# feixue94/pram

Hardware: AMD Instinct MI355X
Metric: query images/sec (640x480, 2048 kpts, 7Scenes nc113) (higher is better)
Workload: dtype f32 results via split-fp16 MFMA (f16 x3 products, f32 accumulate); 1 GPU; 7Scenes full hot path: SFD2 extract+sample -> SegNetViT nc113 (15 layers) -> GML match + 20 Sinkhorn iters, 2048 query kpts vs a 2048-kpt reference set; stages=erm; precision=x3, batches_in_flight_per_gpu=3, hipgraph_replay=False, attention_chunk_keys=4096, frame=640x480, keypoints=2048, parallelism=query-sharded x1, one all-gather of result records, matches_last_step=14291, matches_correct_last_step=14288, gather_order_verified=True

## Files before the change

include/pram_hip.h:

```cpp
#ifndef PRAM_HIP_H
#define PRAM_HIP_H

#include <stddef.h>
#include <stdint.h>

#ifdef __cplusplus
extern "C" {
#endif

#define PRAM_OK 0
#define PRAM_E_ARG (-1)
#define PRAM_E_LAUNCH (-2)
#define PRAM_E_UNSUPPORTED (-3)

int pram_hip_version(void);
const char* pram_last_error(void);
const char* pram_last_kernel(void);

#define PRAM_STATUS_X3_RANGE 1u
int pram_set_status_word(unsigned int* device_word);
float pram_x3_set_act_scale(float scale);
int pram_read_status_word(unsigned int* host_out, int reset, void* stream);


// ... 194 lines not shown

int pram_sample_nhwc_f32(const float* fmap, int batch, int fh, int fw, int c, const float* kpts,
                         const int* lens, int n_max, int s, int l2norm, float* out, void* stream);


int pram_sfd2_row_list(const float* kpts, const int* lens, int batch, int n_max, int fh, int fw, int s, int* rows,
                       int* n_rows, int* pix2row, int rlen, void* stream);

int pram_conv3x3_rows_x3_f32(const float* in, int batch, int h, int w, int cin, const void* wgt_hi, const void* wgt_lo,
                             float w_scale, const float* bias, const int* rows, const int* n_rows, int rlen, float* out,
                             int cout, int relu, void* stream);

int pram_conv1x1_rows_x3_l2norm_f32(const float* in, int batch, int rlen, int cin, const void* wgt_hi, const void* wgt_lo,
                                    float w_scale, const float* bias, const int* n_rows, float* out, int cout, void* stream);

int pram_sample_rows_f32(const float* rowmap, const int* pix2row, int batch, int rlen, int fh, int fw, int c, const float* kpts,
                         const int* lens, int n_max, int s, int l2norm, float* out, void* stream);

int pram_l2norm_rows_f32(float* x, int rows, int cols, void* stream);

int pram_score_lookup_f32(const float* score_map, long long map_stride, int h, int w, const float* kpts,
                          const int* lens, int batch, int n_max, float* out, void* stream);


int pram_resize_bilinear_f32(const float* in, float* out, int planes, int h, int w, int oh, int ow,
                             void* stream);

int pram_seg_epilogue_f32(const float* logits, const int* lens, int batch, int n_max, int n_class,
                          float bg_threshold, float* seg_scores, int* seg_ids, int* non_bg_mask,
                          int* n_non_bg, void* stream);
// ... 251 lines not shown
```

pram_amd/_lib.py:

```python
from __future__ import annotations

import ctypes as C
from pathlib import Path

import os as _os
_LIB_PATH = Path(_os.environ["PRAM_HIP_LIB"]) if _os.environ.get("PRAM_HIP_LIB") else Path(__file__).resolve().parent / "csrc" / "libpram_hip.so"
_lib = None

P = C.c_void_p
I = C.c_int
F = C.c_float
LL = C.c_longlong
SZ = C.c_size_t

_SIGS = {
    "pram_hip_version": (I, []),
    "pram_last_error": (C.c_char_p, []),
    "pram_last_kernel": (C.c_char_p, []),
    "pram_set_status_word": (I, [P]),
    "pram_read_status_word": (I, [P, I, P]),
    "pram_x3_set_act_scale": (F, [F]),
    "pram_linear_f32": (I, [P, I, I, P, I, I, P, P, P, I, P, I, I, I, F, I, P, P, I, P]),
    "pram_linear_f16_f32": (I, [P, I, I, P, I, I, P, P, P, I, P, I, I, I, F, I, P, P, I, P]),
    "pram_linear_f16_ragged_f32": (I, [P, I, I, P, I, I, P, P, P, I, P, I, I, I, F, I, P, P, I, P, I, P]),
# ... 46 lines not shown
    "pram_conv2d_nhwc_f32": (I, [P, I, I, I, I, P, P, P, P, P, P, I, I, I, I, P]),
    "pram_conv2d_nhwc_f16_f32": (I, [P, I, I, I, I, P, P, P, P, P, P, I, I, I, I, P]),
    "pram_conv3x3_grouped_nhwc_f32": (I, [P, I, I, I, I, P, P, P, P, I, I, P]),
    "pram_image_to_nhwc4_f32": (I, [P, P, I, I, I, P]),
    "pram_nhwc_to_nchw_f32": (I, [P, P, I, I, I, I, P]),
    "pram_score_map_f32": (I, [P, P, I, I, I, P]),
    "pram_simple_nms_workspace_bytes": (SZ, [I, I, I]),
    "pram_simple_nms_f32": (I, [P, P, I, I, I, I, P, P]),
    "pram_select_keypoints_workspace_bytes": (SZ, [I, I, I, I]),
    "pram_select_keypoints_f32": (I, [P, I, I, I, F, I, I, I, I, P, P, P, P, P]),
    "pram_sample_nhwc_f32": (I, [P, I, I, I, I, P, P, I, I, I, P, P]),
    "pram_l2norm_rows_f32": (I, [P, I, I, P]),
    "pram_sfd2_row_list": (I, [P, P, I, I, I, I, I, P, P, P, I, P]),
    "pram_conv3x3_rows_x3_f32": (I, [P, I, I, I, I, P, P, F, P, P, P, I, P, I, I, P]),
    "pram_conv1x1_rows_x3_l2norm_f32": (I, [P, I, I, I, P, P, F, P, P, P, I, P]),
    "pram_sample_rows_f32": (I, [P, P, I, I, I, I, I, P, P, I, I, I, P, P]),
    "pram_resize_bilinear_f32": (I, [P, P, I, I, I, I, I, P]),
    "pram_seg_epilogue_f32": (I, [P, P, I, I, I, F, P, P, P, P, P]),
    "pram_row_sort_desc_f32": (I, [P, I, I, I, P, P, P]),
    "pram_row_top2_f32": (I, [P, I, LL, P, P, I, I, I, I, P, P, P, P]),
    "pram_proj_dist_top2_f32": (I, [P, I, P, P, I, I, F, P, P, P, P]),
    "pram_proj_dist_top2_f64uv": (I, [P, I, P, P, I, I, I, C.c_double, P, P, P, P]),
    "pram_project_points_f64": (I, [P, P, P, I, C.c_double, C.c_double, P, P, P, P, P, P]),
    "pram_seg_vote": (I, [P, P, I, I, I, P, P, P, P, P, P, P]),
    "pram_pack_record_f32": (I, [P, P, P, P, P, I, I, I, P, P]),
    "pram_fill_u32": (I, [P, C.c_uint, SZ, P]),
    "pram_stage_frames_u8": (I, [P, P, P, I, I, I, P]),
    "pram_score_lookup_f32": (I, [P, LL, I, I, P, P, I, I, P, P]),
    "pram_cand_mask_ranks": (I, [P, P, I, I, I, P]),
    "pram_cand_plan": (I, [P, P, P, P, P, I, I, I, I, P, P, P, I, I, P, P, P, P, I, I, C.c_double, I, P, P]),
# ... 80 lines not shown
```

pram_amd/csrc/conv.hip:

```cpp
#include <stdlib.h>
#include "gemm_core.h"
#include "gemm_core_f16.h"
#include "gemm_core_x3.h"
#include "gemm_core_x3w.h"
#include "launch.h"

namespace {

struct ConvArgs {
    const float* in; const float* w; const float* bias; const float* scale; const float* shift;
    const float* residual; float* out;
    int batch, h, wd, cin, cout, ks, stride, relu;
    int ho, wo, m, k;
    int tiles_m, tiles_n;
    unsigned int* status;
    _Float16* out_hi; _Float16* out_lo;
    float act_scale = gemmx3::ACT_SCALE;
    const int* rows = nullptr; const int* n_rows = nullptr; int rlen = 0;
};

constexpr int ROWS_BM = 256;

template <int MI, int WN>
__device__ __forceinline__ void conv_epilogue(const ConvArgs& p, f32x16 (&acc)[MI][2], int row0, int col0, int BM, int BN) {
// ... 31 lines not shown
            }
            if (full) {
#pragma unroll
                for (int e = 0; e < 16; ++e) p.out[(size_t)(rbase + acc_row(mi, e, h)) * p.cout + col] = q[e];
            } else {
#pragma unroll
                for (int e = 0; e < 16; ++e) {
                    const int row = rbase + acc_row(mi, e, h);
                    if (row < p.m && col < p.cout) p.out[(size_t)row * p.cout + col] = q[e];
                }
            }
        }
    }
}

template <int MI, int WN>
__device__ __forceinline__ void conv_epilogue_l2norm(const ConvArgs& p, f32x16 (&acc)[MI][2], int row0, int col0, int BM, float* scratch) {
    using gemm::acc_row;
    const int tid = threadIdx.x;
    const int lane = tid & 63, wave = tid >> 6;
    const int wm = wave / WN, wn = wave % WN;
    const int r = lane & 31, h = lane >> 5;
    const int nlast = p.cout - 1, mlast = p.m - 1;
    const int rloc = wm * 32 * MI;
    const int rbase = row0 + rloc;
#pragma unroll
    for (int ni = 0; ni < 2; ++ni) {
        const int col = col0 + wn * 64 + ni * 32 + r;
        const int cc = min(col, nlast);
        const float bi = p.bias ? p.bias[cc] : 0.f;
        const float sc = p.scale ? p.scale[cc] : 1.f;
        const float sh = p.scale ? p.shift[cc] : 0.f;
#pragma unroll
        for (int mi = 0; mi < MI; ++mi)
#pragma unroll
            for (int e = 0; e < 16; ++e) {
                float v = acc[mi][ni][e] + bi;
                if (p.scale) v = v * sc + sh;
                if (p.residual) v += p.residual[(size_t)min(rbase + acc_row(mi, e, h), mlast) * p.cout + cc];
                if (p.relu) v = fmaxf(v, 0.f);
                acc[mi][ni][e] = col < p.cout ? v : 0.f;
            }
    }
    __syncthreads();
#pragma unroll
    for (int mi = 0; mi < MI; ++mi)
#pragma unroll
        for (int e = 0; e < 16; ++e) {
            float s = acc[mi][0][e] * acc[mi][0][e] + acc[mi][1][e] * acc[mi][1][e];
            s += __builtin_bit_cast(float, __builtin_amdgcn_update_dpp(0, __builtin_bit_cast(int, s), 0xB1, 0xF, 0xF, false));
            s += __builtin_bit_cast(float, __builtin_amdgcn_update_dpp(0, __builtin_bit_cast(int, s), 0x4E, 0xF, 0xF, false));
            s += __builtin_bit_cast(float, __builtin_amdgcn_update_dpp(0, __builtin_bit_cast(int, s), 0x141, 0xF, 0xF, false));
            s += __builtin_bit_cast(float, __builtin_amdgcn_update_dpp(0, __builtin_bit_cast(int, s), 0x140, 0xF, 0xF, false));
            s += __shfl_xor(s, 16, 64);
            if (r == 0) scratch[wn * BM + rloc + acc_row(mi, e, h)] = s;
        }
    __syncthreads();
#pragma unroll
    for (int mi = 0; mi < MI; ++mi)
#pragma unroll
        for (int e = 0; e < 16; ++e) {
            const int tr = rloc + acc_row(mi, e, h);
            float tot = 0.f;
#pragma unroll
            for (int w = 0; w < WN; ++w) tot += scratch[w * BM + tr];
            const float d = fmaxf(sqrtf(tot), 1e-12f);
            const int row = row0 + tr;
#pragma unroll
            for (int ni = 0; ni < 2; ++ni) {
                const int col = col0 + wn * 64 + ni * 32 + r;
                if (row < p.m && col < p.cout) p.out[(size_t)row * p.cout + col] = acc[mi][ni][e] / d;
            }
        }
}

template <int MI, int WN>
__device__ __forceinline__ void conv_epilogue_planes(const ConvArgs& p, f32x16 (&acc)[MI][2], int row0, int col0, int BM, int BN) {
    const int tid = threadIdx.x;
    const int lane = tid & 63, wave = tid >> 6;
    const int wm = wave / WN, wn = wave % WN;
    const int r = lane & 31, h = lane >> 5;
    const int nlast = p.cout - 1, mlast = p.m - 1;
    const int rbase = row0 + wm * 32 * MI;
    const bool full = (row0 + BM <= p.m) && (col0 + BN <= p.cout);
    const bool odd = lane & 1;
    unsigned int* plane = reinterpret_cast<unsigned int*>(odd ? p.out_lo : p.out_hi);
    const unsigned int sel = odd ? 0x03020706u : 0x05040100u;
    const unsigned int hc = (unsigned int)p.cout >> 1;
// ... 220 lines not shown
    auto okb = [&](int pp, int kt) -> bool { return (col0 + brow + 64 * pp) < p.cout; };
    f32x16 acc[MI][2];
    float amax = 0.f;
    mainloop<MI, WN>(smem, adv, la, oka, lb, okb, p.k / BK, p.act_scale, acc, amax);
    x3_range_flag(p.status, amax);
#pragma unroll
    for (int mi = 0; mi < MI; ++mi)
#pragma unroll
        for (int ni = 0; ni < 2; ++ni)
#pragma unroll
            for (int e = 0; e < 16; ++e) acc[mi][ni][e] *= inv;
    if constexpr (L2N) conv_epilogue_l2norm<MI, WN>(p, acc, row0, col0, BM, reinterpret_cast<float*>(&smem));
    else conv_epilogue<MI, WN>(p, acc, row0, col0, BM, BN);
}

template <int MI, int WM, int WN, bool PLANES = false, bool GATHER = false>
__global__ __launch_bounds__(64 * WM * WN, 2) void conv_x3w_kernel(ConvArgs p, const _Float16* __restrict__ wh,
                                                                    const _Float16* __restrict__ wl, float inv) {
    using namespace gemmx3w;
    using C = Cfg<MI, WM, WN>;
    constexpr int BM = C::BM, BN = C::BN;
    extern __shared__ __attribute__((aligned(16))) unsigned char smem_raw[];
    Smem<MI, WM, WN>& smem = *reinterpret_cast<Smem<MI, WM, WN>*>(smem_raw);
    const int nblk = p.tiles_m * p.tiles_n;
    const int id = xcd_remap(blockIdx.x, nblk);
    const int tn = id % p.tiles_n, tm = id / p.tiles_n;
    const int tid = threadIdx.x;
    const int arow = tid >> 3, akq = tid & 7, qrow = tid >> 2, qsl = tid & 3;
    const int row0 = tm * BM, col0 = tn * BN;
    const int pad = p.ks >> 1;
    int seg = 0, seg_row0 = 0, live = 0;
// ... 44 lines not shown
        const unsigned off = in ? (unsigned)(roff[pp] + tap) : 0u;
        return *reinterpret_cast<const float4*>(base[pp] + off);
    };
    auto oka = [&](int pp, int kt) -> bool {
        const int iy = iy0[pp] + cky, ix = ix0[pp] + ckx;
        return ok[pp] && (unsigned)iy < (unsigned)p.h && (unsigned)ix < (unsigned)p.wd;
    };
    auto lb = [&](int pp, int kt, int plane) -> uint4 { return *reinterpret_cast<const uint4*>((plane ? wl : wh) + boff[pp] + koff); };
    auto okb = [&](int pp, int kt) -> bool { return (col0 + qrow + C::RQ * pp) < p.cout; };
    f32x16 acc[MI][2];
    auto aptr = [](int, int, int) -> const _Float16* { return nullptr; };
    auto bptr = [&](int row, int plane, int kt) -> const _Float16* {
        return (plane ? wl : wh) + (size_t)min(col0 + row, nlast) * p.k + koff;
    };
    float amax = 0.f;
    mainloop<MI, WM, WN, false, 0, 1>(smem, adv, la, oka, lb, okb, aptr, bptr, p.k / BK, p.act_scale, acc, amax);
    x3_range_flag(p.status, amax);
#pragma unroll
    for (int mi = 0; mi < MI; ++mi)
#pragma unroll
        for (int ni = 0; ni < 2; ++ni)
#pragma unroll
            for (int e = 0; e < 16; ++e) acc[mi][ni][e] *= inv;
    if constexpr (PLANES) conv_epilogue_planes<MI, WN>(p, acc, row0, col0, BM, BN);
    else conv_epilogue<MI, WN>(p, acc, row0, col0, BM, BN);
}

namespace halo {
constexpr int TH = 8, TW = 32, HWD = TW + 2, HHT = TH + 2, HP = HWD * HHT;
constexpr int BK = 32, NT = 512;
constexpr int NL = (HP * 8 + NT - 1) / NT;
template <int WN_>
struct alignas(16) Smem {
    _Float16 ah[2][HP * BK];
    _Float16 al[2][HP * BK];
    _Float16 bh[2][WN_ * 64 * BK];
    _Float16 bl[2][WN_ * 64 * BK];
};
}

template <int WN>
__global__ __launch_bounds__(halo::NT, 1) void conv3x3_x3h_kernel(ConvArgs p, const _Float16* __restrict__ wh, const _Float16* __restrict__ wl,
                                                                  float inv, int tiles_x, int tiles_y) {
    using namespace halo;
    using gemmx3::half4;
    using gemmx3::half8;
    constexpr int BN = WN * 64, MI = TH / (NT / 64 / WN);
    extern __shared__ __attribute__((aligned(16))) unsigned char smem_raw[];
    Smem<WN>& s = *reinterpret_cast<Smem<WN>*>(smem_raw);
    const int nblk = p.tiles_m * p.tiles_n;
    const int id = xcd_remap(blockIdx.x, nblk);
    const int tn = id % p.tiles_n;
    int t = id / p.tiles_n;
    const int tx = t % tiles_x; t /= tiles_x;
    const int ty = t % tiles_y;
    const int b = t / tiles_y;
// ... 31 lines not shown
            float4 v = hv[j];
            if (!g.inimg) v = make_float4(0.f, 0.f, 0.f, 0.f);
            half4 hi, lo;
            gemmx3::split4(v, p.act_scale, hi, lo, amax);
            if (g.valid) {
                const int off = g.hp * BK + gemmx3::swz(g.q >> 1, g.hp) * 8 + (g.q & 1) * 4;
                *reinterpret_cast<half4*>(&s.ah[buf][off]) = hi;
                *reinterpret_cast<half4*>(&s.al[buf][off]) = lo;
            }
        }
    };
    auto bdma = [&](int buf, int koff) {
        auto bp = [&](int row, int plane) { return (plane ? wl : wh) + (size_t)min(col0 + row, nlast) * p.k + koff; };
        gemmx3w::dma_tile<BN, NT / 64>(s.bh[buf], s.bl[buf], bp);
    };
    f32x16 acc[MI][2];
#pragma unroll
    for (int mi = 0; mi < MI; ++mi)
#pragma unroll
        for (int ni = 0; ni < 2; ++ni)
#pragma unroll
            for (int e = 0; e < 16; ++e) acc[mi][ni][e] = 0.f;
    auto kstep = [&](int abuf, int bbuf, int ky, int kx, int ks) {
        const int brow0 = (wn * 64 + r) * BK;
        const int bslot = gemmx3::swz(2 * ks + h, r) * 8;
        half8 bh[2], bl[2], ah[2], al[2];
#pragma unroll
        for (int ni = 0; ni < 2; ++ni) {
            bh[ni] = *reinterpret_cast<const half8*>(&s.bh[bbuf][brow0 + ni * 32 * BK + bslot]);
            bl[ni] = *reinterpret_cast<const half8*>(&s.bl[bbuf][brow0 + ni * 32 * BK + bslot]);
        }
        auto aoff = [&](int mi) {
            const int hp = (wm * MI + mi + ky) * HWD + r + kx;
            return hp * BK + gemmx3::swz(2 * ks + h, hp) * 8;
        };
        int o = aoff(0);
        ah[0] = *reinterpret_cast<const half8*>(&s.ah[abuf][o]);
        al[0] = *reinterpret_cast<const half8*>(&s.al[abuf][o]);
// ... 8 lines not shown
#pragma unroll
            for (int ni = 0; ni < 2; ++ni) acc[mi][ni] = __builtin_amdgcn_mfma_f32_32x32x16_f16(al[mi & 1], bh[ni], acc[mi][ni], 0, 0, 0);
#pragma unroll
            for (int ni = 0; ni < 2; ++ni) acc[mi][ni] = __builtin_amdgcn_mfma_f32_32x32x16_f16(ah[mi & 1], bl[ni], acc[mi][ni], 0, 0, 0);
#pragma unroll
            for (int ni = 0; ni < 2; ++ni) acc[mi][ni] = __builtin_amdgcn_mfma_f32_32x32x16_f16(ah[mi & 1], bh[ni], acc[mi][ni], 0, 0, 0);
        }
    };
    const int nslab = p.cin / BK;
    hload(0);
    bdma(0, 0);
    hcommit(0);
    asm volatile("s_waitcnt vmcnt(0)" ::: "memory");
    __syncthreads();
    int c = 0;
    for (int slab = 0; slab < nslab; ++slab) {
        const bool more_slab = slab + 1 < nslab;
#pragma unroll 1
        for (int tap = 0; tap < 9; ++tap, ++c) {
            const int ky = tap / 3, kx = tap - ky * 3;
            const bool more = tap < 8 || more_slab;
            if (more) {
                const int nt = tap < 8 ? tap + 1 : 0, ns = tap < 8 ? slab : slab + 1;
                bdma((c + 1) & 1, nt * p.cin + ns * BK);
            }
            const bool fetch = tap == 0 && more_slab;
            if (fetch) hload(slab + 1);
            __builtin_amdgcn_sched_barrier(0);
            kstep(slab & 1, c & 1, ky, kx, 0);
            kstep(slab & 1, c & 1, ky, kx, 1);
            __builtin_amdgcn_sched_barrier(0);
            if (tap == 8 && more_slab) hcommit((slab + 1) & 1);
            if (fetch) asm volatile("s_waitcnt vmcnt(%0)" ::"n"(NL) : "memory");
            else asm volatile("s_waitcnt vmcnt(0)" ::: "memory");
            __syncthreads();
        }
    }
    x3_range_flag(p.status, amax);
    const int rbase = wm * 32 * MI;
    float* out_b = p.out + (size_t)b * p.ho * p.wo * p.cout;
    const float* res_b = p.residual ? p.residual + (size_t)b * p.ho * p.wo * p.cout : nullptr;
#pragma unroll
    for (int ni = 0; ni < 2; ++ni) {
        const int col = col0 + wn * 64 + ni * 32 + r;
        const int cc = min(col, nlast);
        const float bi = p.bias ? p.bias[cc] : 0.f;
        const float sc = p.scale ? p.scale[cc] : 1.f;
        const float sh = p.scale ? p.shift[cc] : 0.f;
#pragma unroll
        for (int mi = 0; mi < MI; ++mi)
#pragma unroll
            for (int e = 0; e < 16; ++e) {
                const int tr = rbase + gemm::acc_row(mi, e, h);
                const int oy = oy0 + (tr >> 5), ox = ox0 + (tr & 31);
                if (oy < p.ho && ox < p.wo && col < p.cout) {
// ... 325 lines not shown
    PRAM_REQUIRE(batch >= 0 && rlen > 0 && rlen % ROWS_BM == 0 && (long long)batch * rlen < (1ll << 31),
                 "%s: rlen=%d must be a positive multiple of %d (batch * rlen < 2^31)", who, rlen, ROWS_BM);
    p.batch = 1; p.h = 1; p.wd = batch * rlen; p.cin = cin; p.cout = cout; p.ks = 1; p.stride = 1; p.relu = 0;
    if (int e = conv_args(who, p, CONV_X3, in && wgt_hi && wgt_lo && out && n_rows, w_scale)) return e;
    PRAM_REQUIRE(cout > 0 && cout <= 128, "%s: cout=%d must be at most 128", who, cout);
    if (batch == 0) return PRAM_OK;
    const float inv = arm_split(p, w_scale);
    p.n_rows = n_rows; p.rlen = rlen;
    p.tiles_m = cdiv(p.m, gemmx3::Cfg<2, 2>::BM);
    p.tiles_n = 1;
    hipLaunchKernelGGL((conv_x3_kernel<2, 2, true, true>), dim3(p.tiles_m), dim3(gemmx3::NT), 0, (hipStream_t)stream, p,
                       (const _Float16*)wgt_hi, (const _Float16*)wgt_lo, inv);
    return pram_launch_status(who);
}

extern "C" int pram_conv2d_nhwc_x3_planes(const float* in, int batch, int h, int w, int cin, const void* wgt_hi, const void* wgt_lo,
                                          float w_scale, const float* bias, const float* scale, const float* shift,
                                          const float* residual, void* out_hi, void* out_lo, int cout, int ks, int stride, int relu,
                                          void* stream) {
    const char* who = "pram_conv2d_nhwc_x3_planes";
    ConvArgs p{};
    p.in = in; p.bias = bias; p.scale = scale; p.shift = shift; p.residual = residual;
    p.batch = batch; p.h = h; p.wd = w; p.cin = cin; p.cout = cout; p.ks = ks; p.stride = stride; p.relu = relu;
    if (int e = conv_args(who, p, CONV_X3, in && wgt_hi && wgt_lo && out_hi && out_lo, w_scale)) return e;
    PRAM_REQUIRE(cout > 0 && cout % 2 == 0, "%s: cout=%d must be even", who, cout);
    if (batch == 0) return PRAM_OK;
    const float inv = arm_split(p, w_scale);
    p.out_hi = (_Float16*)out_hi;
    p.out_lo = (_Float16*)out_lo;
    using CW = gemmx3w::Cfg<4, 2, 4>;
// ... 226 lines not shown
```

pram_amd/nets/sfd2.py:

```python
from __future__ import annotations

from typing import Dict, List, Optional

import torch
import torch.nn as nn

from .. import ops
from . import _blocks as blk

RGB_mean = [0.485, 0.456, 0.406]
RGB_std = [0.229, 0.224, 0.225]


def norm_RGB(img: torch.Tensor) -> torch.Tensor:
    mean = img.new_tensor(RGB_mean).view(-1, 1, 1)
    std = img.new_tensor(RGB_std).view(-1, 1, 1)
    return (img - mean) / std


def _conv_bn(cin, cout, stride=1):
    return nn.Sequential(nn.Conv2d(cin, cout, 3, stride, 1), nn.BatchNorm2d(cout), nn.ReLU(inplace=True))


class _Res(nn.Module):
# ... 50 lines not shown
            P[name + ".s"], P[name + ".t"] = self._bn(sd, name + ".1")
        for i in range(3):
            p = f"conv4.{i}"
            for j in (1, 2, 3):
                P[f"{p}.w{j}"] = self._ohwi(sd[f"{p}.conv{j}.weight"])
                P[f"{p}.s{j}"], P[f"{p}.t{j}"] = self._bn(sd, f"{p}.bn{j}")
        for head in ("convPa", "convDa"):
            P[head + ".w0"] = self._ohwi(sd[head + ".0.weight"])
            P[head + ".b0"] = sd[head + ".0.bias"].float()
            P[head + ".s0"], P[head + ".t0"] = self._bn(sd, head + ".1")
            P[head + ".w3"] = self._ohwi(sd[head + ".3.weight"])
            P[head + ".b3"] = sd[head + ".3.bias"].float()
        for head in ("convPb", "convDb"):
            P[head + ".w"] = self._ohwi(sd[head + ".weight"])
            P[head + ".b"] = sd[head + ".bias"].float()
        return {k: v.contiguous().to(dev) for k, v in P.items()}

    def _backbone(self, image: torch.Tensor):
        blk.require_cuda(image, "ResNet4x")
        P = self._packed_get(self._build_packed)
        fused1 = ops.gemm_prec() in ("x3", "f16")
        x = image.float().contiguous() if fused1 and image.shape[-1] != 4 else ops.image_to_nhwc4(image.float())

        def cbr(x, n, stride=1):
            return ops.conv2d_nhwc(x, P[n + ".w"], P[n + ".b"], P[n + ".s"], P[n + ".t"], ks=3, stride=stride, relu=True)

        if fused1:
            o1b = ops.sfd2_conv1(x, P["conv1a.w"], P["conv1a.b"], P["conv1a.s"], P["conv1a.t"],
                                 P["conv1b.w"], P["conv1b.b"], P["conv1b.s"], P["conv1b.t"])
        else:
# ... 6 lines not shown
            if ops.GROUPED_X3 and ops.gemm_prec() == "x3" and o4.shape[-1] % 64 == 0 and o4.numel() < (1 << 29):
                yh, yl = ops.conv2d_nhwc_planes(o4, P[p + ".w1"], None, P[p + ".s1"], P[p + ".t1"], ks=1, relu=True)
                y = ops.conv3x3_grouped_planes(yh, yl, P[p + ".w2"], P[p + ".s2"], P[p + ".t2"], groups=o4.shape[-1] // 8, relu=True)
            else:
                y = ops.conv2d_nhwc(o4, P[p + ".w1"], None, P[p + ".s1"], P[p + ".t1"], ks=1, relu=True)
                y = ops.conv3x3_grouped_nhwc(y, P[p + ".w2"], P[p + ".s2"], P[p + ".t2"], groups=32, relu=True)
            o4 = ops.conv2d_nhwc(y, P[p + ".w3"], None, P[p + ".s3"], P[p + ".t3"], residual=o4, ks=1, relu=True)
        return P, o1b, o2b, o3b, o4

    def _score_head(self, P, o4):
        pa = ops.conv2d_nhwc(o4, P["convPa.w0"], P["convPa.b0"], P["convPa.s0"], P["convPa.t0"], ks=3, stride=2, relu=True)
        pa = ops.conv2d_nhwc(pa, P["convPa.w3"], P["convPa.b3"], ks=3)
        logits = ops.conv2d_nhwc(pa, P["convPb.w"], P["convPb.b"], ks=1)
        return logits, ops.score_map(logits)

    def _desc_stem(self, P, o4):
        return ops.conv2d_nhwc(o4, P["convDa.w0"], P["convDa.b0"], P["convDa.s0"], P["convDa.t0"], ks=3, relu=True)

    def _desc_head(self, P, o4):
        da = ops.conv2d_nhwc(self._desc_stem(P, o4), P["convDa.w3"], P["convDa.b3"], ks=3)
        return ops.conv2d_nhwc(da, P["convDb.w"], P["convDb.b"], ks=1, l2norm=True)

    @staticmethod
    def _nchw_view(x_nhwc: torch.Tensor) -> torch.Tensor:
        return x_nhwc.permute(0, 3, 1, 2)

    @torch.no_grad()
    @blk.with_model_precision
    def det(self, x):
        P, _, _, _, o4 = self._backbone(x)
        _, score = self._score_head(P, o4)
        return score, self._nchw_view(self._desc_head(P, o4))

    @torch.no_grad()
# ... 17 lines not shown
        _, score = self._score_head(P, o4)
        if score.shape[1] != ih or score.shape[2] != iw:
            score = ops.resize_bilinear(score, ih, iw)
        nms = ops.simple_nms(score, 4)
        if cfg['max_keypoints'] < 0:
            kpts, scores, counts = ops.select_keypoints(nms, cfg['conf_th'], cfg['min_keypoints'], cfg['remove_borders'],
                                                        ih * iw, -1 if per_image_fallback else 0)
            k_eff = max(int(counts.max().item()), 1)
            kpts, scores = kpts[:, :k_eff].contiguous(), scores[:, :k_eff].contiguous()
        else:
            kpts, scores, counts = ops.select_keypoints(nms, cfg['conf_th'], cfg['min_keypoints'], cfg['remove_borders'],
                                                        cfg['max_keypoints'], -1 if per_image_fallback else 0)
        if not dense_desc and cfg['max_keypoints'] >= 0 and ops.gemm_prec() == "x3":
            desc_map = None
            descs = ops.sampled_descriptors(self._desc_stem(P, o4), P["convDa.w3"], P["convDa.b3"], P["convDb.w"], P["convDb.b"],
                                            kpts, counts, 4)
        else:
            desc_map = self._desc_head(P, o4)
            descs = ops.sample_nhwc(desc_map, kpts, counts, 4, True)
        return dict(score_map=score, desc_map=desc_map, mid_features=o4, global_nhwc=[o1b, o2b, o3b, o4],
                    keypoints=kpts, scores=scores, descriptors=descs, counts=counts)

    @torch.no_grad()
    def extract_local_global(self, data, config={'conf_th': 0.005, 'remove_borders': 4, 'min_keypoints': 128,
                                                 'max_keypoints': 4096}):
        r = self.extract_batched(data['image'], config, per_image_fallback=False)
        counts: List[int] = r['counts'].tolist()
        return {
            'score_map': r['score_map'],
            'desc_map': self._nchw_view(r['desc_map']),
            'mid_features': self._nchw_view(r['mid_features']),
# ... 128 lines not shown
```

pram_amd/ops.py:

```python
from __future__ import annotations

from typing import Optional, Tuple

import torch

from . import _lib

_INT64 = torch.int64


def _st() -> int:
    return torch.cuda.current_stream().cuda_stream


def _p(t: Optional[torch.Tensor]) -> Optional[int]:
    return None if t is None else t.data_ptr()


def _chk(t: torch.Tensor, name: str, dtype=torch.float32):
    if not t.is_cuda:
        raise _lib.PramHipError(f"{name}: expected a CUDA tensor (pram_amd has no CPU path)")
    if t.dtype != dtype:
        raise _lib.PramHipError(f"{name}: expected {dtype}, got {t.dtype}")

# ... 995 lines not shown
    _lib.check(L.pram_sample_nhwc_f32(_p(fmap), B, fh, fw, Cc, _p(kpts), _p(lens), N, int(s), int(l2norm), _p(out), _st()),
               "pram_sample_nhwc_f32")
    return out


SPARSE_DESC_MAX_FRACTION = 0.9
SPARSE_ROWS_TILE = 256


def sparse_desc_rows(n_max: int, fh: int, fw: int) -> int:
    r = -(-min(4 * n_max, fh * fw) // SPARSE_ROWS_TILE) * SPARSE_ROWS_TILE
    return r if 0 < r < SPARSE_DESC_MAX_FRACTION * fh * fw and fh * fw <= (1 << 18) else 0


def sparse_descriptors(x: torch.Tensor, w3: torch.Tensor, b3, w1: torch.Tensor, b1, kpts: torch.Tensor, lens: Optional[torch.Tensor],
                       s: int, rlen: int, want_parts: bool = False):
    L = _lib.load()
    _chk(x, "x")
    assert x.is_contiguous() and w3.is_contiguous() and w1.is_contiguous()
    kpts = kpts.contiguous()
    B, fh, fw, Cin = x.shape
    N = kpts.shape[1]
    Cm, Cout = w3.shape[0], w1.shape[0]
    dev = x.device
    rows = torch.empty(B, rlen, device=dev, dtype=torch.int32)
    n_rows = torch.empty(B, device=dev, dtype=torch.int32)
    pix2row = torch.empty(B, fh * fw, device=dev, dtype=torch.int32)
    _lib.check(L.pram_sfd2_row_list(_p(kpts), _p(lens), B, N, fh, fw, int(s), _p(rows), _p(n_rows), _p(pix2row), rlen, _st()),
               "pram_sfd2_row_list")
    mid = torch.empty(B * rlen, Cm, device=dev, dtype=torch.float32)
    wh, wl, ws = split_weight(w3)
    _lib.check(L.pram_conv3x3_rows_x3_f32(_p(x), B, fh, fw, Cin, _p(wh), _p(wl), ws, _p(b3), _p(rows), _p(n_rows), rlen, _p(mid), Cm, 0,
                                          _st()), "pram_conv3x3_rows_x3_f32")
    dmat = torch.empty(B * rlen, Cout, device=dev, dtype=torch.float32)
    wh, wl, ws = split_weight(w1)
    _lib.check(L.pram_conv1x1_rows_x3_l2norm_f32(_p(mid), B, rlen, Cm, _p(wh), _p(wl), ws, _p(b1), _p(n_rows), _p(dmat), Cout, _st()),
               "pram_conv1x1_rows_x3_l2norm_f32")
    out = _filled((B, N, Cout), dev)
    _lib.check(L.pram_sample_rows_f32(_p(dmat), _p(pix2row), B, rlen, fh, fw, Cout, _p(kpts), _p(lens), N, int(s), 1, _p(out), _st()),
               "pram_sample_rows_f32")
    return (out, rows, n_rows, pix2row) if want_parts else out


def sampled_descriptors(x: torch.Tensor, w3: torch.Tensor, b3, w1: torch.Tensor, b1, kpts: torch.Tensor, lens: Optional[torch.Tensor],
                        s: int) -> torch.Tensor:
    rlen = sparse_desc_rows(kpts.shape[1], x.shape[1], x.shape[2]) if FUSED_L2NORM else 0
    if rlen:
        return sparse_descriptors(x, w3, b3, w1, b1, kpts, lens, s, rlen)
    dm = conv2d_nhwc(conv2d_nhwc(x, w3, b3, ks=3, precision="x3"), w1, b1, ks=1, precision="x3", l2norm=True)
    return sample_nhwc(dm, kpts, lens, s, True)


def l2norm_rows_(x: torch.Tensor) -> torch.Tensor:
    L = _lib.load()
    assert x.is_contiguous()
    cols = x.shape[-1]
    _lib.check(L.pram_l2norm_rows_f32(_p(x), x.numel() // cols, cols, _st()), "pram_l2norm_rows_f32")
    return x


def score_lookup(score_map_: torch.Tensor, kpts: torch.Tensor, lens: Optional[torch.Tensor]) -> torch.Tensor:
    L = _lib.load()
    score_map_ = score_map_.contiguous()
    kpts = kpts.contiguous()
    B, H, W = score_map_.shape
# ... 1021 lines not shown
```

Baseline: 613.2 queries/s.

## Fold descriptor 3x3 and 1x1 head convs into one conv with fused L2 norm

The linear 3x3 conv (convDa.w3, no ReLU) followed by the 1x1 conv convDb is algebraically folded into a single 3x3 conv. Weights and bias are combined in double precision at load time. New kernels (a dense halo head and a sparse rows variant) run this folded conv with an L2-normalise epilogue, split the K reduction into two accumulators, and add an output range check. This removes the intermediate mid-channel map, one kernel launch and its memory traffic. In exchange the folded conv has K = 9*Cin feeding Cout outputs, which may mean more MACs if Cm is small relative to Cout, and rounding changes under split-fp16.

```diff
diff --git a/include/pram_hip.h b/include/pram_hip.h
--- a/include/pram_hip.h
+++ b/include/pram_hip.h
@@ -232,6 +232,14 @@
 int pram_conv1x1_rows_x3_l2norm_f32(const float* in, int batch, int rlen, int cin, const void* wgt_hi, const void* wgt_lo,
                                     float w_scale, const float* bias, const int* n_rows, float* out, int cout, void* stream);
 
+
+int pram_conv3x3_head_x3_f32(const float* in, int batch, int h, int w, int cin, const void* wgt_hi, const void* wgt_lo,
+                             float w_scale, const float* bias, float* out, int cout, void* stream);
+
+int pram_conv3x3_rows_x3_l2norm_f32(const float* in, int batch, int h, int w, int cin, const void* wgt_hi, const void* wgt_lo,
+                                    float w_scale, const float* bias, const int* rows, const int* n_rows, int rlen, float* out,
+                                    int cout, void* stream);
+
 int pram_sample_rows_f32(const float* rowmap, const int* pix2row, int batch, int rlen, int fh, int fw, int c, const float* kpts,
                          const int* lens, int n_max, int s, int l2norm, float* out, void* stream);
 
diff --git a/pram_amd/_lib.py b/pram_amd/_lib.py
--- a/pram_amd/_lib.py
+++ b/pram_amd/_lib.py
@@ -84,6 +84,8 @@
     "pram_sfd2_row_list": (I, [P, P, I, I, I, I, I, P, P, P, I, P]),
     "pram_conv3x3_rows_x3_f32": (I, [P, I, I, I, I, P, P, F, P, P, P, I, P, I, I, P]),
     "pram_conv1x1_rows_x3_l2norm_f32": (I, [P, I, I, I, P, P, F, P, P, P, I, P]),
+    "pram_conv3x3_head_x3_f32": (I, [P, I, I, I, I, P, P, F, P, P, I, P]),
+    "pram_conv3x3_rows_x3_l2norm_f32": (I, [P, I, I, I, I, P, P, F, P, P, P, I, P, I, P]),
     "pram_sample_rows_f32": (I, [P, P, I, I, I, I, I, P, P, I, I, I, P, P]),
     "pram_resize_bilinear_f32": (I, [P, P, I, I, I, I, I, P]),
     "pram_seg_epilogue_f32": (I, [P, P, I, I, I, F, P, P, P, P, P]),
diff --git a/pram_amd/csrc/conv.hip b/pram_amd/csrc/conv.hip
--- a/pram_amd/csrc/conv.hip
+++ b/pram_amd/csrc/conv.hip
@@ -69,7 +69,47 @@
     }
 }
 
-template <int MI, int WN>
+template <int MI, int WN, class OutRow>
+__device__ __forceinline__ void l2norm_rows_store(f32x16 (&acc)[MI][2], int cout, int col0, int BM, float* scratch, OutRow& outrow) {
+    using gemm::acc_row;
+    const int tid = threadIdx.x;
+    const int lane = tid & 63, wave = tid >> 6;
+    const int wm = wave / WN, wn = wave % WN;
+    const int r = lane & 31, h = lane >> 5;
+    const int rloc = wm * 32 * MI;
+    __syncthreads();
+#pragma unroll
+    for (int mi = 0; mi < MI; ++mi)
+#pragma unroll
+        for (int e = 0; e < 16; ++e) {
+            float s = acc[mi][0][e] * acc[mi][0][e] + acc[mi][1][e] * acc[mi][1][e];
+            s += __builtin_bit_cast(float, __builtin_amdgcn_update_dpp(0, __builtin_bit_cast(int, s), 0xB1, 0xF, 0xF, false));
+            s += __builtin_bit_cast(float, __builtin_amdgcn_update_dpp(0, __builtin_bit_cast(int, s), 0x4E, 0xF, 0xF, false));
+            s += __builtin_bit_cast(float, __builtin_amdgcn_update_dpp(0, __builtin_bit_cast(int, s), 0x141, 0xF, 0xF, false));
+            s += __builtin_bit_cast(float, __builtin_amdgcn_update_dpp(0, __builtin_bit_cast(int, s), 0x140, 0xF, 0xF, false));
+            s += __shfl_xor(s, 16, 64);
+            if (r == 0) scratch[wn * BM + rloc + acc_row(mi, e, h)] = s;
+        }
+    __syncthreads();
+#pragma unroll
+    for (int mi = 0; mi < MI; ++mi)
+#pragma unroll
+        for (int e = 0; e < 16; ++e) {
+            const int tr = rloc + acc_row(mi, e, h);
+            float tot = 0.f;
+#pragma unroll
+            for (int w = 0; w < WN; ++w) tot += scratch[w * BM + tr];
+            const float d = fmaxf(sqrtf(tot), 1e-12f);
+            float* dst = outrow(tr);
+#pragma unroll
+            for (int ni = 0; ni < 2; ++ni) {
+                const int col = col0 + wn * 64 + ni * 32 + r;
+                if (dst != nullptr && col < cout) dst[col] = acc[mi][ni][e] / d;
+            }
+        }
+}
+
+template <int MI, int WN, bool GUARD = false>
 __device__ __forceinline__ void conv_epilogue_l2norm(const ConvArgs& p, f32x16 (&acc)[MI][2], int row0, int col0, int BM, float* scratch) {
     using gemm::acc_row;
     const int tid = threadIdx.x;
@@ -79,6 +119,7 @@
     const int nlast = p.cout - 1, mlast = p.m - 1;
     const int rloc = wm * 32 * MI;
     const int rbase = row0 + rloc;
+    float omax = 0.f;
 #pragma unroll
     for (int ni = 0; ni < 2; ++ni) {
         const int col = col0 + wn * 64 + ni * 32 + r;
@@ -95,38 +136,12 @@
                 if (p.residual) v += p.residual[(size_t)min(rbase + acc_row(mi, e, h), mlast) * p.cout + cc];
                 if (p.relu) v = fmaxf(v, 0.f);
                 acc[mi][ni][e] = col < p.cout ? v : 0.f;
-            }
-    }
-    __syncthreads();
-#pragma unroll
-    for (int mi = 0; mi < MI; ++mi)
-#pragma unroll
-        for (int e = 0; e < 16; ++e) {
-            float s = acc[mi][0][e] * acc[mi][0][e] + acc[mi][1][e] * acc[mi][1][e];
-            s += __builtin_bit_cast(float, __builtin_amdgcn_update_dpp(0, __builtin_bit_cast(int, s), 0xB1, 0xF, 0xF, false));
-            s += __builtin_bit_cast(float, __builtin_amdgcn_update_dpp(0, __builtin_bit_cast(int, s), 0x4E, 0xF, 0xF, false));
-            s += __builtin_bit_cast(float, __builtin_amdgcn_update_dpp(0, __builtin_bit_cast(int, s), 0x141, 0xF, 0xF, false));
-            s += __builtin_bit_cast(float, __builtin_amdgcn_update_dpp(0, __builtin_bit_cast(int, s), 0x140, 0xF, 0xF, false));
-            s += __shfl_xor(s, 16, 64);
-            if (r == 0) scratch[wn * BM + rloc + acc_row(mi, e, h)] = s;
-        }
-    __syncthreads();
-#pragma unroll
-    for (int mi = 0; mi < MI; ++mi)
-#pragma unroll
-        for (int e = 0; e < 16; ++e) {
-            const int tr = rloc + acc_row(mi, e, h);
-            float tot = 0.f;
-#pragma unroll
-            for (int w = 0; w < WN; ++w) tot += scratch[w * BM + tr];
-            const float d = fmaxf(sqrtf(tot), 1e-12f);
-            const int row = row0 + tr;
-#pragma unroll
-            for (int ni = 0; ni < 2; ++ni) {
-                const int col = col0 + wn * 64 + ni * 32 + r;
-                if (row < p.m && col < p.cout) p.out[(size_t)row * p.cout + col] = acc[mi][ni][e] / d;
-            }
-        }
+                if constexpr (GUARD) omax = fmaxf(omax, fabsf(acc[mi][ni][e]));
+            }
+    }
+    if constexpr (GUARD) x3_range_flag(p.status, omax * p.act_scale);
+    auto outrow = [&](int tr) -> float* { return row0 + tr < p.m ? p.out + (size_t)(row0 + tr) * p.cout : nullptr; };
+    l2norm_rows_store<MI, WN>(acc, p.cout, col0, BM, scratch, outrow);
 }
 
 template <int MI, int WN>
@@ -377,7 +392,7 @@
     else conv_epilogue<MI, WN>(p, acc, row0, col0, BM, BN);
 }
 
-template <int MI, int WM, int WN, bool PLANES = false, bool GATHER = false>
+template <int MI, int WM, int WN, bool PLANES = false, bool GATHER = false, bool L2N = false>
 __global__ __launch_bounds__(64 * WM * WN, 2) void conv_x3w_kernel(ConvArgs p, const _Float16* __restrict__ wh,
                                                                     const _Float16* __restrict__ wl, float inv) {
     using namespace gemmx3w;
@@ -452,7 +467,25 @@
         return (plane ? wl : wh) + (size_t)min(col0 + row, nlast) * p.k + koff;
     };
     float amax = 0.f;
-    mainloop<MI, WM, WN, false, 0, 1>(smem, adv, la, oka, lb, okb, aptr, bptr, p.k / BK, p.act_scale, acc, amax);
+    if constexpr (L2N) {
+        const int half = p.cin / BK / 2;
+        const int nk0 = half * p.ks * p.ks;
+        mainloop<MI, WM, WN, false, 0, 1>(smem, adv, la, oka, lb, okb, aptr, bptr, nk0, p.act_scale, acc, amax);
+        auto adv1 = [&](int kt) {
+            if (kt == 0) { cky = ckx = 0; cci = half * BK; koff = cci; tap = cci; return; }
+            adv(kt);
+        };
+        f32x16 acc1[MI][2];
+        mainloop<MI, WM, WN, false, 0, 1>(smem, adv1, la, oka, lb, okb, aptr, bptr, p.k / BK - nk0, p.act_scale, acc1, amax);
+#pragma unroll
+        for (int mi = 0; mi < MI; ++mi)
+#pragma unroll
+            for (int ni = 0; ni < 2; ++ni)
+#pragma unroll
+                for (int e = 0; e < 16; ++e) acc[mi][ni][e] += acc1[mi][ni][e];
+    } else {
+        mainloop<MI, WM, WN, false, 0, 1>(smem, adv, la, oka, lb, okb, aptr, bptr, p.k / BK, p.act_scale, acc, amax);
+    }
     x3_range_flag(p.status, amax);
 #pragma unroll
     for (int mi = 0; mi < MI; ++mi)
@@ -460,7 +493,8 @@
         for (int ni = 0; ni < 2; ++ni)
 #pragma unroll
             for (int e = 0; e < 16; ++e) acc[mi][ni][e] *= inv;
-    if constexpr (PLANES) conv_epilogue_planes<MI, WN>(p, acc, row0, col0, BM, BN);
+    if constexpr (L2N) conv_epilogue_l2norm<MI, WN, true>(p, acc, row0, col0, BM, reinterpret_cast<float*>(smem_raw));
+    else if constexpr (PLANES) conv_epilogue_planes<MI, WN>(p, acc, row0, col0, BM, BN);
     else conv_epilogue<MI, WN>(p, acc, row0, col0, BM, BN);
 }
 
@@ -477,7 +511,7 @@
 };
 }
 
-template <int WN>
+template <int WN, bool HEAD = false>
 __global__ __launch_bounds__(halo::NT, 1) void conv3x3_x3h_kernel(ConvArgs p, const _Float16* __restrict__ wh, const _Float16* __restrict__ wl,
                                                                   float inv, int tiles_x, int tiles_y) {
     using namespace halo;
@@ -539,14 +573,14 @@
         auto bp = [&](int row, int plane) { return (plane ? wl : wh) + (size_t)min(col0 + row, nlast) * p.k + koff; };
         gemmx3w::dma_tile<BN, NT / 64>(s.bh[buf], s.bl[buf], bp);
     };
-    f32x16 acc[MI][2];
+    f32x16 acc[MI][2], acc1[MI][2];
 #pragma unroll
     for (int mi = 0; mi < MI; ++mi)
 #pragma unroll
         for (int ni = 0; ni < 2; ++ni)
 #pragma unroll
-            for (int e = 0; e < 16; ++e) acc[mi][ni][e] = 0.f;
-    auto kstep = [&](int abuf, int bbuf, int ky, int kx, int ks) {
+            for (int e = 0; e < 16; ++e) acc[mi][ni][e] = acc1[mi][ni][e] = 0.f;
+    auto kstep = [&](f32x16 (&acc)[MI][2], int abuf, int bbuf, int ky, int kx, int ks) {
         const int brow0 = (wn * 64 + r) * BK;
         const int bslot = gemmx3::swz(2 * ks + h, r) * 8;
         half8 bh[2], bl[2], ah[2], al[2];
@@ -585,31 +619,62 @@
     asm volatile("s_waitcnt vmcnt(0)" ::: "memory");
     __syncthreads();
     int c = 0;
-    for (int slab = 0; slab < nslab; ++slab) {
-        const bool more_slab = slab + 1 < nslab;
+    auto slabs = [&](f32x16 (&A)[MI][2], int s0, int s1) {
+        for (int slab = s0; slab < s1; ++slab) {
+            const bool more_slab = slab + 1 < nslab;
 #pragma unroll 1
-        for (int tap = 0; tap < 9; ++tap, ++c) {
-            const int ky = tap / 3, kx = tap - ky * 3;
-            const bool more = tap < 8 || more_slab;
-            if (more) {
-                const int nt = tap < 8 ? tap + 1 : 0, ns = tap < 8 ? slab : slab + 1;
-                bdma((c + 1) & 1, nt * p.cin + ns * BK);
-            }
-            const bool fetch = tap == 0 && more_slab;
-            if (fetch) hload(slab + 1);
-            __builtin_amdgcn_sched_barrier(0);
-            kstep(slab & 1, c & 1, ky, kx, 0);
-            kstep(slab & 1, c & 1, ky, kx, 1);
-            __builtin_amdgcn_sched_barrier(0);
-            if (tap == 8 && more_slab) hcommit((slab + 1) & 1);
-            if (fetch) asm volatile("s_waitcnt vmcnt(%0)" ::"n"(NL) : "memory");
-            else asm volatile("s_waitcnt vmcnt(0)" ::: "memory");
-            __syncthreads();
-        }
+            for (int tap = 0; tap < 9; ++tap, ++c) {
+                const int ky = tap / 3, kx = tap - ky * 3;
+                const bool more = tap < 8 || more_slab;
+                if (more) {
+                    const int nt = tap < 8 ? tap + 1 : 0, ns = tap < 8 ? slab : slab + 1;
+                    bdma((c + 1) & 1, nt * p.cin + ns * BK);
+                }
+                const bool fetch = tap == 0 && more_slab;
+                if (fetch) hload(slab + 1);
+                __builtin_amdgcn_sched_barrier(0);
+                kstep(A, slab & 1, c & 1, ky, kx, 0);
+                kstep(A, slab & 1, c & 1, ky, kx, 1);
+                __builtin_amdgcn_sched_barrier(0);
+                if (tap == 8 && more_slab) hcommit((slab + 1) & 1);
+                if (fetch) asm volatile("s_waitcnt vmcnt(%0)" ::"n"(NL) : "memory");
+                else asm volatile("s_waitcnt vmcnt(0)" ::: "memory");
+                __syncthreads();
+            }
+        }
+    };
+    if constexpr (HEAD) {
+        slabs(acc, 0, nslab / 2);
+        slabs(acc1, nslab / 2, nslab);
+    } else {
+        slabs(acc, 0, nslab);
     }
     x3_range_flag(p.status, amax);
     const int rbase = wm * 32 * MI;
     float* out_b = p.out + (size_t)b * p.ho * p.wo * p.cout;
+    if constexpr (HEAD) {
+        float omax = 0.f;
+#pragma unroll
+        for (int ni = 0; ni < 2; ++ni) {
+            const int col = col0 + wn * 64 + ni * 32 + r;
+            const float bi = p.bias ? p.bias[min(col, nlast)] : 0.f;
+#pragma unroll
+            for (int mi = 0; mi < MI; ++mi)
+#pragma unroll
+                for (int e = 0; e < 16; ++e) {
+                    const float v = (acc[mi][ni][e] + acc1[mi][ni][e]) * inv + bi;
+                    acc[mi][ni][e] = col < p.cout ? v : 0.f;
+                    omax = fmaxf(omax, fabsf(acc[mi][ni][e]));
+                }
+        }
+        x3_range_flag(p.status, omax * p.act_scale);
+        auto outrow = [&](int tr) -> float* {
+            const int oy = oy0 + (tr >> 5), ox = ox0 + (tr & 31);
+            return oy < p.ho && ox < p.wo ? out_b + (size_t)(oy * p.wo + ox) * p.cout : nullptr;
+        };
+        l2norm_rows_store<MI, WN>(acc, p.cout, col0, TH * TW, reinterpret_cast<float*>(smem_raw), outrow);
+        return;
+    }
     const float* res_b = p.residual ? p.residual + (size_t)b * p.ho * p.wo * p.cout : nullptr;
 #pragma unroll
     for (int ni = 0; ni < 2; ++ni) {
@@ -965,6 +1030,54 @@
     return pram_launch_status(who);
 }
 
+extern "C" int pram_conv3x3_head_x3_f32(const float* in, int batch, int h, int w, int cin, const void* wgt_hi, const void* wgt_lo,
+                                        float w_scale, const float* bias, float* out, int cout, void* stream) {
+    const char* who = "pram_conv3x3_head_x3_f32";
+    ConvArgs p{};
+    p.in = in; p.bias = bias; p.out = out;
+    p.batch = batch; p.h = h; p.wd = w; p.cin = cin; p.cout = cout; p.ks = 3; p.stride = 1; p.relu = 0;
+    if (int e = conv_args(who, p, CONV_X3, in && wgt_hi && wgt_lo && out, w_scale)) return e;
+    PRAM_REQUIRE(cin % 64 == 0, "%s: cin=%d must be a multiple of 64 (two halves of whole 32-channel slabs)", who, cin);
+    PRAM_REQUIRE(cout > 0 && cout <= 128, "%s: cout=%d must be at most 128", who, cout);
+    PRAM_REQUIRE((long long)p.ho * p.wo * cout < (1ll << 31), "%s: a map of %d x %d x %d elements does not fit 32-bit offsets", who, p.ho, p.wo, cout);
+    if (batch == 0) return PRAM_OK;
+    const float inv = arm_split(p, w_scale);
+    const int tiles_x = cdiv(p.wo, halo::TW), tiles_y = cdiv(p.ho, halo::TH);
+    p.tiles_m = batch * tiles_x * tiles_y;
+    p.tiles_n = 1;
+    hipStream_t st = (hipStream_t)stream;
+    const _Float16* wh = (const _Float16*)wgt_hi;
+    const _Float16* wl = (const _Float16*)wgt_lo;
+    opt_in_lds<conv3x3_x3h_kernel<2, true>>(sizeof(halo::Smem<2>));
+    hipLaunchKernelGGL((conv3x3_x3h_kernel<2, true>), dim3(p.tiles_m), dim3(halo::NT), sizeof(halo::Smem<2>), st, p, wh, wl, inv, tiles_x, tiles_y);
+    return pram_launch_status(who);
+}
+
+extern "C" int pram_conv3x3_rows_x3_l2norm_f32(const float* in, int batch, int h, int w, int cin, const void* wgt_hi, const void* wgt_lo,
+                                               float w_scale, const float* bias, const int* rows, const int* n_rows, int rlen, float* out,
+                                               int cout, void* stream) {
+    const char* who = "pram_conv3x3_rows_x3_l2norm_f32";
+    ConvArgs p{};
+    p.in = in; p.bias = bias; p.out = out;
+    p.batch = batch; p.h = h; p.wd = w; p.cin = cin; p.cout = cout; p.ks = 3; p.stride = 1; p.relu = 0;
+    if (int e = conv_args(who, p, CONV_X3, in && wgt_hi && wgt_lo && out && rows && n_rows, w_scale)) return e;
+    PRAM_REQUIRE(cin % 64 == 0, "%s: cin=%d must be a multiple of 64 (two halves of whole 32-channel slabs)", who, cin);
+    PRAM_REQUIRE(cout > 0 && cout <= 128, "%s: cout=%d must be at most 128", who, cout);
+    PRAM_REQUIRE(rlen > 0 && rlen % ROWS_BM == 0 && (long long)batch * rlen < (1ll << 31),
+                 "%s: rlen=%d must be a positive multiple of %d (batch * rlen < 2^31)", who, rlen, ROWS_BM);
+    if (batch == 0) return PRAM_OK;
+    const float inv = arm_split(p, w_scale);
+    p.rows = rows; p.n_rows = n_rows; p.rlen = rlen;
+    p.m = batch * rlen;
+    using CW = gemmx3w::Cfg<2, 4, 2>;
+    static_assert(CW::BM == ROWS_BM && CW::BN == 128, "ROWS_BM is this tile's height");
+    const size_t shm = sizeof(gemmx3w::Smem<2, 4, 2>);
+    opt_in_lds<conv_x3w_kernel<2, 4, 2, false, true, true>>(shm);
+    hipLaunchKernelGGL((conv_x3w_kernel<2, 4, 2, false, true, true>), dim3(set_tiles<CW>(p, cout)), dim3(CW::NT), shm, (hipStream_t)stream, p,
+                       (const _Float16*)wgt_hi, (const _Float16*)wgt_lo, inv);
+    return pram_launch_status(who);
+}
+
 extern "C" int pram_conv2d_nhwc_x3_planes(const float* in, int batch, int h, int w, int cin, const void* wgt_hi, const void* wgt_lo,
                                           float w_scale, const float* bias, const float* scale, const float* shift,
                                           const float* residual, void* out_hi, void* out_lo, int cout, int ks, int stride, int relu,
diff --git a/pram_amd/nets/sfd2.py b/pram_amd/nets/sfd2.py
--- a/pram_amd/nets/sfd2.py
+++ b/pram_amd/nets/sfd2.py
@@ -88,6 +88,7 @@
         for head in ("convPb", "convDb"):
             P[head + ".w"] = self._ohwi(sd[head + ".weight"])
             P[head + ".b"] = sd[head + ".bias"].float()
+        P["convD.wf"], P["convD.bf"] = ops.fold_head(P["convDa.w3"], P["convDa.b3"], P["convDb.w"], P["convDb.b"])
         return {k: v.contiguous().to(dev) for k, v in P.items()}
 
     def _backbone(self, image: torch.Tensor):
@@ -124,10 +125,16 @@
         logits = ops.conv2d_nhwc(pa, P["convPb.w"], P["convPb.b"], ks=1)
         return logits, ops.score_map(logits)
 
+    @staticmethod
+    def _folded() -> bool:
+        return ops.HEAD_FOLD and ops.gemm_prec() == "x3"
+
     def _desc_stem(self, P, o4):
         return ops.conv2d_nhwc(o4, P["convDa.w0"], P["convDa.b0"], P["convDa.s0"], P["convDa.t0"], ks=3, relu=True)
 
     def _desc_head(self, P, o4):
+        if self._folded():
+            return ops.conv3x3_head(self._desc_stem(P, o4), P["convD.wf"], P["convD.bf"])
         da = ops.conv2d_nhwc(self._desc_stem(P, o4), P["convDa.w3"], P["convDa.b3"], ks=3)
         return ops.conv2d_nhwc(da, P["convDb.w"], P["convDb.b"], ks=1, l2norm=True)
 
@@ -175,7 +182,7 @@
         if not dense_desc and cfg['max_keypoints'] >= 0 and ops.gemm_prec() == "x3":
             desc_map = None
             descs = ops.sampled_descriptors(self._desc_stem(P, o4), P["convDa.w3"], P["convDa.b3"], P["convDb.w"], P["convDb.b"],
-                                            kpts, counts, 4)
+                                            kpts, counts, 4, folded=(P["convD.wf"], P["convD.bf"]) if self._folded() else None)
         else:
             desc_map = self._desc_head(P, o4)
             descs = ops.sample_nhwc(desc_map, kpts, counts, 4, True)
diff --git a/pram_amd/ops.py b/pram_amd/ops.py
--- a/pram_amd/ops.py
+++ b/pram_amd/ops.py
@@ -1033,7 +1033,10 @@
 
 
 def sparse_descriptors(x: torch.Tensor, w3: torch.Tensor, b3, w1: torch.Tensor, b1, kpts: torch.Tensor, lens: Optional[torch.Tensor],
-                       s: int, rlen: int, want_parts: bool = False):
+                       s: int, rlen: int, want_parts: bool = False, folded=None):
+    if folded is not None:
+        r = folded_sparse_descriptors(x, folded[0], folded[1], kpts, lens, s, rlen, want_parts)
+        return r[:4] if want_parts else r
     L = _lib.load()
     _chk(x, "x")
     assert x.is_contiguous() and w3.is_contiguous() and w1.is_contiguous()
@@ -1062,12 +1065,62 @@
 
 
 def sampled_descriptors(x: torch.Tensor, w3: torch.Tensor, b3, w1: torch.Tensor, b1, kpts: torch.Tensor, lens: Optional[torch.Tensor],
-                        s: int) -> torch.Tensor:
+                        s: int, folded=None) -> torch.Tensor:
     rlen = sparse_desc_rows(kpts.shape[1], x.shape[1], x.shape[2]) if FUSED_L2NORM else 0
     if rlen:
-        return sparse_descriptors(x, w3, b3, w1, b1, kpts, lens, s, rlen)
+        return sparse_descriptors(x, w3, b3, w1, b1, kpts, lens, s, rlen, folded=folded)
+    if folded is not None:
+        return sample_nhwc(conv3x3_head(x, folded[0], folded[1]), kpts, lens, s, True)
     dm = conv2d_nhwc(conv2d_nhwc(x, w3, b3, ks=3, precision="x3"), w1, b1, ks=1, precision="x3", l2norm=True)
     return sample_nhwc(dm, kpts, lens, s, True)
+
+
+HEAD_FOLD = True
+
+
+def fold_head(w3: torch.Tensor, b3: torch.Tensor, w1: torch.Tensor, b1: torch.Tensor):
+    m = w1.reshape(w1.shape[0], -1).double()
+    w = torch.einsum("om,mhwc->ohwc", m, w3.double())
+    b = m @ b3.double() + b1.double()
+    return w.float().contiguous(), b.float().contiguous()
+
+
+def conv3x3_head(x: torch.Tensor, w: torch.Tensor, bias: torch.Tensor) -> torch.Tensor:
+    L = _lib.load()
+    _chk(x, "x")
+    assert x.is_contiguous() and w.is_contiguous() and tuple(w.shape[1:3]) == (3, 3)
+    B, H, W, Cin = x.shape
+    Cout = w.shape[0]
+    out = torch.empty(B, H, W, Cout, device=x.device, dtype=torch.float32)
+    wh, wl, ws = split_weight(w)
+    _lib.check(L.pram_conv3x3_head_x3_f32(_p(x), B, H, W, Cin, _p(wh), _p(wl), ws, _p(bias), _p(out), Cout, _st()),
+               "pram_conv3x3_head_x3_f32")
+    return out
+
+
+def folded_sparse_descriptors(x: torch.Tensor, w: torch.Tensor, bias: torch.Tensor, kpts: torch.Tensor, lens: Optional[torch.Tensor],
+                              s: int, rlen: int, want_parts: bool = False):
+    L = _lib.load()
+    _chk(x, "x")
+    assert x.is_contiguous() and w.is_contiguous()
+    kpts = kpts.contiguous()
+    B, fh, fw, Cin = x.shape
+    N = kpts.shape[1]
+    Cout = w.shape[0]
+    dev = x.device
+    rows = torch.empty(B, rlen, device=dev, dtype=torch.int32)
+    n_rows = torch.empty(B, device=dev, dtype=torch.int32)
+    pix2row = torch.empty(B, fh * fw, device=dev, dtype=torch.int32)
+    _lib.check(L.pram_sfd2_row_list(_p(kpts), _p(lens), B, N, fh, fw, int(s), _p(rows), _p(n_rows), _p(pix2row), rlen, _st()),
+               "pram_sfd2_row_list")
+    dmat = torch.empty(B * rlen, Cout, device=dev, dtype=torch.float32)
+    wh, wl, ws = split_weight(w)
+    _lib.check(L.pram_conv3x3_rows_x3_l2norm_f32(_p(x), B, fh, fw, Cin, _p(wh), _p(wl), ws, _p(bias), _p(rows), _p(n_rows), rlen, _p(dmat),
+                                                 Cout, _st()), "pram_conv3x3_rows_x3_l2norm_f32")
+    out = _filled((B, N, Cout), dev)
+    _lib.check(L.pram_sample_rows_f32(_p(dmat), _p(pix2row), B, rlen, fh, fw, Cout, _p(kpts), _p(lens), N, int(s), 1, _p(out), _st()),
+               "pram_sample_rows_f32")
+    return (out, rows, n_rows, pix2row, dmat) if want_parts else out
 
 
 def l2norm_rows_(x: torch.Tensor) -> torch.Tensor:
```

Result: no change. 618.4 queries/s, median of 6 (+0.8%).
